# Paleogenomics/pss-bam

Measured on AMD Instinct MI355X. Metric: aligned reads/s (whole node) + HBM GB/s fraction, 200M x 150bp BAM, higher is better.
Workload: dtype u64

## Files before the change

### include/pssbam_hip.h

```cpp
#ifndef PSSBAM_HIP_H
#define PSSBAM_HIP_H

#include <stddef.h>
#include <stdint.h>

#ifdef __cplusplus
extern "C" {
#endif

#define PSSBAM_ABI_VERSION 1
#define PSSBAM_MAX_KLEN 15
#define PSSBAM_MAX_READ_GROUPS 4096
#define PSSBAM_MAX_LENGTH_BINS 64
#define PSSBAM_MAX_CONTIG_SETS 4096
#define PSSBAM_MAX_REPLICATES 64
#define PSSBAM_MAX_MISMATCHES 255
#define PSSBAM_MAX_INTERIOR_MARGIN 65535
#define PSSBAM_MAX_COMPOSITION 30
#define PSSBAM_MAX_SCORE_DIST 64
#define PSSBAM_MAX_SCORE_QUAL 64
#define PSSBAM_MAX_SCORE_WEIGHT 2047
#define PSSBAM_MAX_SCORE_HALF 128
#define PSSBAM_MAX_HIST_LENGTH 65535
#define PSSBAM_MAX_BASE_QUALITY 93
// ... 209 lines not shown
    uint32_t isize;
    uint64_t out_off;
    uint32_t crc;
    uint32_t status;
} pssbam_bgzf_block;

int64_t pssbam_bgzf_scan(const void *bytes, uint64_t nbytes, pssbam_bgzf_block *blocks, uint64_t max_blocks,
                         uint64_t *consumed, uint64_t *inflated_bytes);

int pssbam_bgzf_inflate_device(void *hip_stream, const void *d_comp, uint64_t comp_bytes, pssbam_bgzf_block *d_blocks,
                               uint32_t n_blocks, void *d_out, int check_crc);

int pssbam_engine_submit_bgzf(pssbam_engine *e, const void *comp, uint64_t comp_bytes, const pssbam_bgzf_block *blocks,
                              uint32_t n_blocks, uint32_t first_record_offset, uint64_t *ticket);
int pssbam_engine_wait_bgzf_copied(pssbam_engine *e, uint64_t ticket);
int pssbam_engine_feed_open(pssbam_engine *e, int32_t n_ref, uint64_t genome_bytes_hint);
int pssbam_engine_feed_break(pssbam_engine *e);
int pssbam_engine_feed_handoff(pssbam_engine *from, pssbam_engine *to);
#define PSSBAM_FEED_BAD_BLOCK 1u
#define PSSBAM_FEED_RAGGED 2u
#define PSSBAM_FEED_BAD_RECORD 4u
#define PSSBAM_FEED_TRUNCATED 8u
int pssbam_engine_feed_status(pssbam_engine *e, uint32_t *flags, double *inflate_ms, uint64_t *inflated_bytes);
int pssbam_engine_hint_records(pssbam_engine *e, const void *records, uint64_t nbytes);
int pssbam_feed_reserve(int device);
int pssbam_feed_release(int device);

int pssbam_bgzf_inflate_host(int device, const void *bgzf, uint64_t nbytes, void *out, uint64_t out_cap, uint64_t *out_len,
                             uint32_t *n_blocks, uint32_t *first_bad_block, uint32_t *first_bad_status, double *kernel_ms,
                             int check_crc, int repeats);

uint64_t pssbam_bgzf_deflate_work_bytes(uint64_t raw_bytes);
int pssbam_bgzf_deflate_device(void *hip_stream, const void *d_raw, uint64_t raw_bytes, void *d_bgzf, uint64_t bgzf_cap,
                               uint64_t *d_totals, void *d_work, uint64_t work_bytes);

int pssbam_bgzf_deflate_host(int device, const void *raw, uint64_t nbytes, void *out, uint64_t out_cap, uint64_t *out_len,
                             uint32_t *n_blocks, double *kernel_ms, int repeats);

int64_t pssbam_index_records(const void *bytes, uint64_t nbytes, uint32_t *offsets,
                             uint64_t max_records, uint64_t *consumed);

#ifdef __cplusplus
}
#endif
#endif
```

### pss-bam_amd/__init__.py

```python
from __future__ import annotations

import ctypes as C
import subprocess
from dataclasses import dataclass
from pathlib import Path

import numpy as np

PKG_DIR = Path(__file__).resolve().parent
ROOT = PKG_DIR.parent
LIB_HIP = PKG_DIR / "libpssbam_hip.so"
LIB_HOST = PKG_DIR / "libpssbam_host.so"
LIB_SYNTH = PKG_DIR / "libpssbam_synth.so"

TALLY_PSS, TALLY_KMER = 1, 2
KERNEL_AUTO, KERNEL_SIMPLE, KERNEL_TILED = 0, 1, 2
ST_NAMES = ["records", "rg_dropped", "parse_skip", "no_contig", "pss_ok", "pss_filtered", "kmer_ok",
            "kmer_filtered", "kmer_fail", "slow_path"]
ST_N = 16

HIP_SYMBOLS = [
    "pssbam_last_error", "pssbam_device_count", "pssbam_warmup", "pssbam_engine_create", "pssbam_engine_destroy",
    "pssbam_engine_set_stream", "pssbam_engine_set_genome", "pssbam_engine_set_genome_arrays",
    "pssbam_engine_set_references", "pssbam_engine_submit", "pssbam_engine_submit_async", "pssbam_engine_wait_copied",
    "pssbam_engine_copy_done", "pssbam_engine_phase_times", "pssbam_engine_submit_device", "pssbam_engine_sync",
    "pssbam_engine_finish", "pssbam_engine_reset", "pssbam_engine_counters_device", "pssbam_engine_bind_counters",
    "pssbam_reduce_counters", "pssbam_engine_genome_kmer_count", "pssbam_host_register", "pssbam_host_unregister", "pssbam_engine_timer_begin",
    "pssbam_engine_timer_end", "pssbam_engine_kernel_time", "pssbam_index_records", "pssbam_bgzf_scan",
    "pssbam_bgzf_inflate_device", "pssbam_bgzf_inflate_host", "pssbam_engine_submit_bgzf", "pssbam_engine_wait_bgzf_copied",
    "pssbam_engine_feed_status", "pssbam_engine_feed_break", "pssbam_engine_feed_handoff", "pssbam_feed_reserve", "pssbam_engine_hint_records",
    "pssbam_engine_set_genome_async", "pssbam_engine_genome_wait", "pssbam_engine_feed_open", "pssbam_feed_release",
    "pssbam_engine_set_read_groups", "pssbam_engine_finish_groups", "pssbam_engine_set_length_bins",
    "pssbam_engine_set_contig_sets", "pssbam_engine_finish_kmer_groups", "pssbam_engine_set_min_base_quality",
    "pssbam_engine_set_regions", "pssbam_engine_set_length_histogram", "pssbam_engine_finish_length_histogram",
    "pssbam_engine_set_site_context", "pssbam_engine_finish_site_context",
    "pssbam_engine_set_end_condition", "pssbam_engine_finish_end_condition", "pssbam_engine_set_gapped_reads",
    "pssbam_engine_set_per_contig", "pssbam_engine_finish_contigs",
    "pssbam_engine_set_mismatches", "pssbam_engine_finish_mismatches", "pssbam_engine_set_replicates",
    "pssbam_engine_set_interior", "pssbam_engine_finish_interior",
    "pssbam_engine_set_composition", "pssbam_engine_finish_composition",
    "pssbam_engine_set_read_score", "pssbam_engine_finish_read_score",
    "pssbam_engine_set_record_sink", "pssbam_engine_set_block_sink", "pssbam_engine_set_end_mask",
    "pssbam_engine_set_duplicates", "pssbam_engine_finish_duplicates",
    "pssbam_engine_set_coverage", "pssbam_engine_finish_coverage", "pssbam_engine_finish_coverage_runs",
    "pssbam_engine_set_sites", "pssbam_engine_finish_sites",
    "pssbam_bgzf_deflate_work_bytes", "pssbam_bgzf_deflate_device", "pssbam_bgzf_deflate_host",
]
MAX_READ_GROUPS = 4096
MAX_LENGTH_BINS = 64
MAX_CONTIG_SETS = 4096
MAX_REPLICATES = 64
MAX_BASE_QUALITY = 93
MAX_HIST_LENGTH = 65535
# ... 764 lines not shown
            rc = L.pssbam_engine_submit_bgzf(self._h, bgzf.ctypes.data + base_in, end_in - base_in, grp, j - i, skip, C.byref(t))
            if rc == EBUSY and on_busy is not None:
                on_busy()
                rc = L.pssbam_engine_submit_bgzf(self._h, bgzf.ctypes.data + base_in, end_in - base_in, grp, j - i, skip, C.byref(t))
            _chk(rc)
            _chk(L.pssbam_engine_wait_bgzf_copied(self._h, t.value))
            skip = 0
            i = j
        return int(n)

    def feed_break(self):
        self._L.pssbam_engine_feed_break.argtypes = [C.c_void_p]
        _chk(self._L.pssbam_engine_feed_break(self._h))

    def feed_handoff(self, to: "Engine"):
        self._L.pssbam_engine_feed_handoff.argtypes = [C.c_void_p, C.c_void_p]
        _chk(self._L.pssbam_engine_feed_handoff(self._h, to._h))

    def feed_status(self) -> dict:
        L = self._L
        L.pssbam_engine_feed_status.argtypes = [C.c_void_p, C.POINTER(C.c_uint32), C.POINTER(C.c_double), C.POINTER(C.c_uint64)]
        f, ms, nb = C.c_uint32(), C.c_double(), C.c_uint64()
        _chk(L.pssbam_engine_feed_status(self._h, C.byref(f), C.byref(ms), C.byref(nb)))
        return {"flags": int(f.value), "inflate_ms": float(ms.value), "inflated_bytes": int(nb.value)}

    def submit_device(self, d_records: int, nbytes: int, d_offsets: int, n_records: int):
        _chk(self._L.pssbam_engine_submit_device(self._h, C.c_void_p(d_records), nbytes, C.c_void_p(d_offsets),
                                                 n_records))

    def sync(self):
        _chk(self._L.pssbam_engine_sync(self._h))

    def reset(self):
        _chk(self._L.pssbam_engine_reset(self._h))

    def finish(self) -> Tables:
        fwd = rev = k5 = k3 = None
        if self.has_pss:
            fwd = np.zeros((self.region_len + 2, 16), dtype=np.uint64)
            rev = np.zeros_like(fwd)
        if self.has_kmer:
            k5 = np.zeros(4 ** self.klen, dtype=np.uint64)
            k3 = np.zeros_like(k5)
        st = np.zeros(ST_N, dtype=np.uint64)
        p = lambda a: a.ctypes.data if a is not None else None
        _chk(self._L.pssbam_engine_finish(self._h, p(fwd), p(rev), p(k5), p(k3), st.ctypes.data))
        return Tables(fwd, rev, k5, k3, {n: int(st[i]) for i, n in enumerate(ST_NAMES)})
# ... 96 lines not shown
```

### pss-bam_amd/csrc/bgzf_api.h

```cpp
#pragma once

#include "inflate_kernels.h"
#include "inflate_wave.h"

extern "C" int64_t pssbam_bgzf_scan(const void *bytes, uint64_t nbytes, pssbam_bgzf_block *blocks, uint64_t max_blocks,
                                    uint64_t *consumed, uint64_t *inflated_bytes) {
    const uint8_t *p = (const uint8_t *)bytes;
    uint64_t o = 0, n = 0, uoff = 0;
    while (o + 18 <= nbytes && (!blocks || n < max_blocks)) {
        if (p[o] != 0x1f || p[o + 1] != 0x8b || p[o + 2] != 8 || !(p[o + 3] & 4)) { fail(PSSBAM_EFORMAT, "not a BGZF block at offset %llu", (unsigned long long)o); return PSSBAM_EFORMAT; }
        const uint32_t xlen = p[o + 10] | ((uint32_t)p[o + 11] << 8);
        if (o + 12 + xlen > nbytes) break;
        uint32_t bsize = 0;
        bool found = false;
        for (uint32_t x = 0; x + 4 <= xlen;) {
            const uint8_t *sf = p + o + 12 + x;
            const uint32_t slen = sf[2] | ((uint32_t)sf[3] << 8);
            if (sf[0] == 'B' && sf[1] == 'C' && slen == 2 && x + 6 <= xlen) { bsize = (sf[4] | ((uint32_t)sf[5] << 8)) + 1u; found = true; break; }
            x += 4 + slen;
        }
        if (!found || bsize < 12u + xlen + 8u) { fail(PSSBAM_EFORMAT, "BGZF block at offset %llu has no usable BC field", (unsigned long long)o); return PSSBAM_EFORMAT; }
        if (o + bsize > nbytes) break;
        uint32_t crc, isize;
        memcpy(&crc, p + o + bsize - 8, 4);
        memcpy(&isize, p + o + bsize - 4, 4);
        if (isize > 65536u) { fail(PSSBAM_EFORMAT, "BGZF ISIZE %u exceeds 64 KiB", isize); return PSSBAM_EFORMAT; }
// ... 100 lines not shown
        if (!crc2_attr_set[dev & 63]) {
            HIP_TRY(hipFuncSetAttribute((const void *)pssbam::bgzf_crc_lines_kernel, hipFuncAttributeMaxDynamicSharedMemorySize, (int)pssbam::CRC2_LDS_BYTES));
            crc2_attr_set[dev & 63] = true;
        }
        const uint32_t cgrid = std::min<uint32_t>((n_blocks + 15) / 16, (uint32_t)n_cu);
        hipLaunchKernelGGL(pssbam::bgzf_crc_lines_kernel, dim3(cgrid), dim3(1024), pssbam::CRC2_LDS_BYTES, st, (const uint8_t *)d_out, (pssbam::BgzfBlock *)d_blocks, n_blocks,
                           (const uint32_t *)xpow16, (const uint32_t *)ztab);
        HIP_TRY(hipGetLastError());
        return PSSBAM_OK;
    }
    if (beside_inflate) {
        const uint32_t cgrid = std::min<uint32_t>((n_blocks + 3) / 4, (uint32_t)n_cu);
        hipLaunchKernelGGL(pssbam::bgzf_crc_kernel<4u>, dim3(cgrid), dim3(256), 4u * 256u * 4u * 4u, st, (const uint8_t *)d_out, (pssbam::BgzfBlock *)d_blocks, n_blocks, xpow);
    } else {
        static const uint32_t crc_waves = getenv("PSSBAM_CRC_WAVES") ? (uint32_t)std::min(16, std::max(1, atoi(getenv("PSSBAM_CRC_WAVES")))) : 16u;
        const uint32_t cgrid = std::min<uint32_t>((n_blocks + crc_waves - 1) / crc_waves, (uint32_t)n_cu);
        hipLaunchKernelGGL(pssbam::bgzf_crc_kernel<pssbam::CRC_REP>, dim3(cgrid), dim3(64 * crc_waves), pssbam::CRC_LDS_BYTES, st, (const uint8_t *)d_out, (pssbam::BgzfBlock *)d_blocks, n_blocks, xpow);
    }
    HIP_TRY(hipGetLastError());
    return PSSBAM_OK;
}

static int launch_inflate(hipStream_t st, const void *d_comp, uint64_t comp_bytes, pssbam_bgzf_block *d_blocks, uint32_t n_blocks,
                          void *d_out, int check_crc, int loop, uint64_t out_bytes, const WaveBufs *wb = nullptr) {
    if (!n_blocks) return PSSBAM_OK;
    if (!d_comp || !d_blocks || !d_out) return fail(PSSBAM_EINVAL, "null buffer");
    if ((uintptr_t)d_comp & 3u) return fail(PSSBAM_EINVAL, "d_comp must be 4-byte aligned");
    int dev = 0, n_cu = 0;
    HIP_TRY(hipGetDevice(&dev));
    HIP_TRY(hipDeviceGetAttribute(&n_cu, hipDeviceAttributeMultiprocessorCount, dev));
    static bool attr_set[64] = {false};
    if (!attr_set[dev & 63]) {
        HIP_TRY(hipFuncSetAttribute((const void *)pssbam::bgzf_inflate_kernel<false>, hipFuncAttributeMaxDynamicSharedMemorySize, (int)pssbam::INF_LDS_BYTES));
        HIP_TRY(hipFuncSetAttribute((const void *)pssbam::bgzf_inflate_kernel<true>, hipFuncAttributeMaxDynamicSharedMemorySize, (int)pssbam::INF_LDS_BYTES_DEFER));
        HIP_TRY(hipFuncSetAttribute((const void *)pssbam::bgzf_inflate_kernel<true, true>, hipFuncAttributeMaxDynamicSharedMemorySize, (int)pssbam::INF_LDS_BYTES_DEFER));
        HIP_TRY(hipFuncSetAttribute((const void *)pssbam::bgzf_inflate_kernel<true, true, true>, hipFuncAttributeMaxDynamicSharedMemorySize, (int)pssbam::INF_LDS_BYTES_DEFER));
        HIP_TRY(hipFuncSetAttribute((const void *)pssbam::bgzf_inflate_kernel<true, false, true>, hipFuncAttributeMaxDynamicSharedMemorySize, (int)pssbam::INF_LDS_BYTES_DEFER));
        attr_set[dev & 63] = true;
    }
    if (loop == -2) loop = 0;
    else if (const char *lm = getenv("PSSBAM_INFLATE_LOOP")) loop = atoi(lm) != 0;
    if (comp_bytes < 64u) loop = 0;
    const uint32_t groups = (n_blocks + pssbam::INF_WAVE - 1) / pssbam::INF_WAVE;
    const char *gm = getenv("PSSBAM_INFLATE_WAVES_PER_CU");
    const uint32_t per_cu = gm && atoi(gm) > 0 ? (uint32_t)atoi(gm) : (uint32_t)pssbam::INF_WAVES_PER_CU;
    const uint32_t grid = std::min<uint32_t>(groups, (uint32_t)n_cu * per_cu);
    uint32_t lit_run = out_bytes && out_bytes >= 8ull * comp_bytes ? 4u : 8u;
// ... 10 lines not shown
            if (!d_dbg2) HIP_TRY(hipMalloc(&d_dbg2, 20 * sizeof(unsigned long long)));
            HIP_TRY(hipMemsetAsync(d_dbg2, 0, 20 * sizeof(unsigned long long), st));
            d_wdbg = d_dbg2;
        }
        hipLaunchKernelGGL(pssbam::bgzf_tokens_kernel, dim3(tgrid), dim3(64 * pssbam::WV_WAVES), 0, st, (const uint8_t *)d_comp, comp_bytes, (pssbam::BgzfBlock *)d_blocks,
                           n_blocks, (uint8_t *)d_out, wb->seq_arena, wb->seq_off, wb->seq_count, d_wdbg);
        const char *rg = getenv("PSSBAM_RESOLVE_WGS_PER_CU");
        const uint32_t rgrid = std::min<uint32_t>((n_blocks + pssbam::RS_WAVES - 1) / pssbam::RS_WAVES, (uint32_t)n_cu * (rg && atoi(rg) > 0 ? (uint32_t)atoi(rg) : 4u));
        hipLaunchKernelGGL(pssbam::bgzf_resolve_kernel, dim3(rgrid), dim3(64 * pssbam::RS_WAVES), 0, st, (uint8_t *)d_out, (pssbam::BgzfBlock *)d_blocks, n_blocks,
                           (const uint32_t *)wb->seq_arena, wb->seq_off, (const uint32_t *)wb->seq_count, d_wdbg);
        HIP_TRY(hipGetLastError());
        if (d_wdbg) {
            unsigned long long h[20];
            HIP_TRY(hipMemcpyAsync(h, d_wdbg, sizeof h, hipMemcpyDeviceToHost, st));
            HIP_TRY(hipStreamSynchronize(st));
            const double nb = (double)std::max<unsigned long long>(h[9], 1), rb = (double)std::max<unsigned long long>(h[16], 1);
            fprintf(stderr, "[pssbam] token kernel stamps, shader cycles per BGZF block (%.0f blocks, %.2f chunks each): set-up+stored %.0f, code-length walk %.0f, table builds %.0f, "
                            "walk A1 %.0f, A2 %.0f, path %.0f, B+scans %.0f, C %.0f\n", nb, h[8] / nb, h[0] / nb, h[1] / nb, h[2] / nb, h[3] / nb, h[4] / nb, h[5] / nb, h[6] / nb, h[7] / nb);
            fprintf(stderr, "[pssbam] resolve kernel stamps, shader cycles per BGZF block (%.0f blocks, %.1f batches and %.1f rounds each): window in %.0f, scans %.0f, rounds %.0f, window out %.0f\n",
                    rb, h[14] / rb, h[15] / rb, h[10] / rb, h[11] / rb, h[12] / rb, h[13] / rb);
        }
        only_status = pssbam::INF_RETRY;
    }
    if (loop > 0 && getenv("PSSBAM_INFLATE_STAMPS")) {
        static unsigned long long *d_dbg = nullptr;
        if (!d_dbg) HIP_TRY(hipMalloc(&d_dbg, 8 * sizeof(unsigned long long)));
        HIP_TRY(hipMemsetAsync(d_dbg, 0, 8 * sizeof(unsigned long long), st));
        if (pieces)
            hipLaunchKernelGGL((pssbam::bgzf_inflate_kernel<true, true, true>), dim3(grid), dim3(pssbam::INF_WAVE), pssbam::INF_LDS_BYTES_DEFER, st, (const uint8_t *)d_comp,
                               comp_bytes, (pssbam::BgzfBlock *)d_blocks, n_blocks, (uint8_t *)d_out, lit_run, d_dbg);
        else
            hipLaunchKernelGGL((pssbam::bgzf_inflate_kernel<true, false, true>), dim3(grid), dim3(pssbam::INF_WAVE), pssbam::INF_LDS_BYTES_DEFER, st, (const uint8_t *)d_comp,
                               comp_bytes, (pssbam::BgzfBlock *)d_blocks, n_blocks, (uint8_t *)d_out, lit_run, d_dbg);
        unsigned long long h[8];
        HIP_TRY(hipMemcpyAsync(h, d_dbg, sizeof h, hipMemcpyDeviceToHost, st));
        HIP_TRY(hipStreamSynchronize(st));
        const double L = (double)std::max<unsigned long long>(h[3], 1);
        fprintf(stderr, "[pssbam] inflate stamps (pieces %d; lane sums, shader cycles): steps %llu, per step: decode %.0f wait %.0f stores+copies %.0f cycles; lanes in a step %.1f of 64; "
                        "literals per step %.2f; steps ending in an in-place copy %.3f; in-loop share of the lanes' kernel cycles %.3f\n", (int)pieces,
                h[3], h[0] / L, h[1] / L, h[2] / L, h[4] / L, h[5] / L, h[6] / L, (double)(h[0] + h[1] + h[2]) / (double)std::max<unsigned long long>(h[7], 1));
    } else if (only_status != 0xFFFFFFFFu && getenv("PSSBAM_INFLATE_WAVE") && atoi(getenv("PSSBAM_INFLATE_WAVE")) == 2) {
    } else if (loop > 0 && pieces)
        hipLaunchKernelGGL((pssbam::bgzf_inflate_kernel<true, true>), dim3(grid), dim3(pssbam::INF_WAVE), pssbam::INF_LDS_BYTES_DEFER, st, (const uint8_t *)d_comp,
                           comp_bytes, (pssbam::BgzfBlock *)d_blocks, n_blocks, (uint8_t *)d_out, lit_run, (unsigned long long *)nullptr, only_status);
    else if (loop > 0)
        hipLaunchKernelGGL(pssbam::bgzf_inflate_kernel<true>, dim3(grid), dim3(pssbam::INF_WAVE), pssbam::INF_LDS_BYTES_DEFER, st, (const uint8_t *)d_comp,
                           comp_bytes, (pssbam::BgzfBlock *)d_blocks, n_blocks, (uint8_t *)d_out, lit_run);
    else
        hipLaunchKernelGGL(pssbam::bgzf_inflate_kernel<false>, dim3(grid), dim3(pssbam::INF_WAVE), pssbam::INF_LDS_BYTES, st, (const uint8_t *)d_comp,
                           comp_bytes, (pssbam::BgzfBlock *)d_blocks, n_blocks, (uint8_t *)d_out, lit_run);
    HIP_TRY(hipGetLastError());
    if (check_crc) return launch_crc(st, d_blocks, n_blocks, d_out);
    return PSSBAM_OK;
}

extern "C" int pssbam_bgzf_inflate_device(void *hip_stream, const void *d_comp, uint64_t comp_bytes, pssbam_bgzf_block *d_blocks,
                                          uint32_t n_blocks, void *d_out, int check_crc) {
    return launch_inflate((hipStream_t)hip_stream, d_comp, comp_bytes, d_blocks, n_blocks, d_out, check_crc, -2, 0);
}


extern "C" int pssbam_bgzf_inflate_host(int device, const void *bgzf, uint64_t nbytes, void *out, uint64_t out_cap, uint64_t *out_len,
                                        uint32_t *n_blocks_out, uint32_t *first_bad_block, uint32_t *first_bad_status, double *kernel_ms,
                                        int check_crc, int repeats) {
    uint64_t consumed = 0, total = 0;
    const int64_t n = pssbam_bgzf_scan(bgzf, nbytes, nullptr, 0, &consumed, &total);
    if (n < 0) return (int)n;
    if (consumed != nbytes) return fail(PSSBAM_EFORMAT, "input ends inside a BGZF block");
    if (out_len) *out_len = total;
    if (n_blocks_out) *n_blocks_out = (uint32_t)n;
    if (first_bad_block) *first_bad_block = 0xFFFFFFFFu;
    if (first_bad_status) *first_bad_status = 0;
    if (n == 0) return PSSBAM_OK;
// ... 437 lines not shown
    HIP_TRY(hipStreamWaitEvent(is, s.copies_done, 0));
    HIP_TRY(hipStreamWaitEvent(is, s.copies_done2, 0));
    if (s.h_blocks_cap < nb) {
        if (s.h_blocks) (void)hipHostFree(s.h_blocks);
        s.h_blocks = nullptr;
        s.h_blocks_cap = 0;
        const size_t cap = std::max<size_t>(nb + nb / 4, 1u << 16);
        if (hipHostMalloc((void **)&s.h_blocks, cap * sizeof(pssbam_bgzf_block), hipHostMallocDefault) == hipSuccess) s.h_blocks_cap = cap;
        else s.h_blocks = nullptr;
    }
    const pssbam_bgzf_block *table = s.blocks.data();
    if (s.h_blocks) {
        memcpy(s.h_blocks, s.blocks.data(), nb * sizeof(pssbam_bgzf_block));
        table = s.h_blocks;
    }
    HIP_TRY(hipMemcpyAsync(s.d_blocks, table, nb * sizeof(pssbam_bgzf_block), hipMemcpyHostToDevice, is));
    hipEvent_t ev0 = take_event(e), ev1 = take_event(e);
    if (!ev0 || !ev1) return fail(PSSBAM_EHIP, "hipEventCreate failed");
    if (!e->feed_base_ev) {
        HIP_TRY(hipEventCreate(&e->feed_base_ev));
        HIP_TRY(hipEventRecord(e->feed_base_ev, is));
    }
    HIP_TRY(hipEventRecord(ev0, is));
    rc = launch_inflate(is, s.d_comp, s.comp_used, (pssbam_bgzf_block *)s.d_blocks, (uint32_t)nb, s.d_out, 0, INFLATE_LOOP_DEFAULT, data_end - FEED_GAP);
    if (rc) return rc;
    if (!s.inflate_done) HIP_TRY(hipEventCreateWithFlags(&s.inflate_done, hipEventDisableTiming));
    HIP_TRY(hipEventRecord(s.inflate_done, is));
    HIP_TRY(hipStreamWaitEvent(e->stream, s.inflate_done, 0));
    if (e->feed_fresh) {
        const uint64_t first = FEED_GAP + e->feed_skip;
        HIP_TRY(hipMemcpyAsync(s.d_chain, &first, sizeof first, hipMemcpyHostToDevice, e->stream));
        e->feed_fresh = false;
    } else {
        hipLaunchKernelGGL(pssbam::bgzf_chain_carry_in, dim3(1), dim3(256), 0, e->stream, (const uint8_t *)e->d_carry, (const uint64_t *)e->d_feed_tail,
                           s.d_out, (uint64_t)FEED_GAP, s.d_chain);
    }
    if (!getenv("PSSBAM_NO_CRC")) {
        rc = launch_crc(e->stream, (pssbam_bgzf_block *)s.d_blocks, (uint32_t)nb, s.d_out, is != e->stream && !getenv("PSSBAM_FEED_BIG_CRC"));
        if (rc) return rc;
    }
    const int32_t n_ref = e->have_refs ? e->n_ref : e->feed_n_ref;
    {
        const uint32_t n = (uint32_t)nb, grid = std::min<uint32_t>((n + 255u) / 256u, (uint32_t)e->n_cu * 8u);
        const pssbam::BgzfBlock *blk = (const pssbam::BgzfBlock *)s.d_blocks;
        hipLaunchKernelGGL(pssbam::bgzf_chain_spec, dim3(grid), dim3(256), 0, e->stream, (const uint8_t *)s.d_out, blk, n, data_end,
                           (const uint64_t *)s.d_chain, n_ref, s.d_a, s.d_n, s.d_e, s.d_last, e->d_feed_flags, s.d_chain + 2);
        hipLaunchKernelGGL(pssbam::bgzf_chain_suffix, dim3(1), dim3(1024), 0, e->stream, (const uint64_t *)s.d_a, n, s.d_nexta, (const uint64_t *)nullptr);
// ... 71 lines not shown
            s.sub_bytes = 0;
        }
        b.in_off = b.in_off - byte0 + comp_at;
        b.out_off = s.out_used;
        b.status = 0;
        s.out_used += b.isize;
        s.sub_bytes += b.isize;
        s.blocks.push_back(b);
    }
    HIP_TRY(hipMemcpyAsync(s.d_comp + comp_at, comp + byte0, byte1 - byte0, hipMemcpyHostToDevice, cs));
    s.comp_used = comp_at + (byte1 - byte0);
    e->h2d_bytes += byte1 - byte0;
    return PSSBAM_OK;
}

static int feed_state_init(pssbam_engine *e) {
    if (e->d_feed_flags) return PSSBAM_OK;
    e->feed_t0 = feed_now();
    if (getenv("PSSBAM_FEED_SUPER_BYTES")) e->feed_out_target = std::max<uint64_t>(1ull << 20, strtoull(getenv("PSSBAM_FEED_SUPER_BYTES"), nullptr, 10));
    if (getenv("PSSBAM_FEED_SUB_BYTES")) e->feed_sub_max = std::min<uint64_t>(FEED_SUB_MAX, std::max<uint64_t>(65536, strtoull(getenv("PSSBAM_FEED_SUB_BYTES"), nullptr, 10)));
    const uint64_t lanes = (uint64_t)e->n_cu * (uint64_t)pssbam::INF_WAVES_PER_CU * 64ull;
    const uint64_t rounds = std::max<uint64_t>(1, e->feed_out_target / (lanes * 65280ull));
    e->feed_block_target = getenv("PSSBAM_FEED_SUPER_BYTES") && e->feed_out_target < lanes * 65280ull ? 0xFFFFFFFFull : rounds * lanes;
    HIP_TRY(hipMalloc(&e->d_feed_flags, sizeof(uint32_t)));
    HIP_TRY(hipMemsetAsync(e->d_feed_flags, 0, sizeof(uint32_t), e->stream));
    HIP_TRY(hipMalloc(&e->d_feed_tail, sizeof(uint64_t)));
    HIP_TRY(hipMemsetAsync(e->d_feed_tail, 0, sizeof(uint64_t), e->stream));
    if (!e->d_carry) HIP_TRY(hipMalloc(&e->d_carry, FEED_GAP));
    if (const char *ib = getenv("PSSBAM_FEED_IDLE_BLOCKS")) e->feed_idle_min_blocks = atoi(ib) > 0 ? (uint64_t)atoi(ib) : ~0ull;
    return PSSBAM_OK;
}

extern "C" int pssbam_engine_feed_open(pssbam_engine *e, int32_t n_ref, uint64_t genome_bytes_hint) {
    if (!e || n_ref < 0) return fail(PSSBAM_EINVAL, "bad argument");
    if (e->cfg.kernel == PSSBAM_KERNEL_SIMPLE) return fail(PSSBAM_EINVAL, "device-indexed blocks need the tiled kernels");
    HIP_TRY(hipSetDevice(e->device));
    if (e->per_contig && !e->have_refs)
        if (const int rc = size_per_contig(e, n_ref)) return rc;
    e->feed_opened = true;
    e->feed_n_ref = n_ref;
    size_t free_b = 0, total_b = 0;
    if (hipMemGetInfo(&free_b, &total_b) == hipSuccess) {
        const uint64_t keep = genome_bytes_hint + genome_bytes_hint / 2 + (8ull << 30) + select_reserve_bytes(e) + dedup_reserve_bytes(e) + coverage_reserve_bytes(e);
        e->feed_mem_budget = e->feed.size() * feed_slot_bytes(e) + (free_b > keep ? free_b - keep : 0);
    }
    return PSSBAM_OK;
}

// ... 141 lines not shown
    to->feed_skip = 0;
    return PSSBAM_OK;
}

extern "C" int pssbam_engine_wait_bgzf_copied(pssbam_engine *e, uint64_t ticket) {
    if (!e) return fail(PSSBAM_EINVAL, "null engine");
    if (!ticket) return PSSBAM_OK;
    for (size_t i = 0; i < e->feed_copies.size(); i++)
        if (e->feed_copies[i].first == ticket) {
            HIP_TRY(hipSetDevice(e->device));
            HIP_TRY(hipEventSynchronize(e->feed_copies[i].second));
            e->feed_event_pool.push_back(e->feed_copies[i].second);
            e->feed_copies.erase(e->feed_copies.begin() + (long)i);
            return PSSBAM_OK;
        }
    return PSSBAM_OK;
}

extern "C" int pssbam_engine_feed_status(pssbam_engine *e, uint32_t *flags, double *inflate_ms, uint64_t *inflated_bytes) {
    if (!e) return fail(PSSBAM_EINVAL, "null engine");
    int rc = pssbam_engine_sync(e);
    if (rc) return rc;
    uint32_t f = 0;
    if (e->d_feed_flags) HIP_TRY(hipMemcpy(&f, e->d_feed_flags, sizeof f, hipMemcpyDeviceToHost));
    if (e->d_feed_tail) {
        uint64_t tail = 0;
        HIP_TRY(hipMemcpy(&tail, e->d_feed_tail, sizeof tail, hipMemcpyDeviceToHost));
        if (tail) f |= pssbam::FEED_TRUNCATED;
    }
    {
        std::vector<std::pair<float, float>> iv;
        for (auto &p : e->inflate_events) {
            float a = 0.f, b = 0.f;
            HIP_TRY(hipEventElapsedTime(&a, e->feed_base_ev, p.first));
            HIP_TRY(hipEventElapsedTime(&b, e->feed_base_ev, p.second));
            iv.emplace_back(a, b);
            e->event_pool.push_back(p.first);
            e->event_pool.push_back(p.second);
        }
        e->inflate_events.clear();
        std::sort(iv.begin(), iv.end());
        float hi = -1e30f;
        for (auto &x : iv) {
            if (x.second <= hi) continue;
            e->inflate_ms += x.second - std::max(x.first, hi);
            hi = x.second;
        }
        if (e->feed_base_ev) { (void)hipEventDestroy(e->feed_base_ev); e->feed_base_ev = nullptr; }
    }
    if (getenv("PSSBAM_STATS"))
        fprintf(stderr, "[pssbam] engine feed: %llu super-batches (%llu cut short because the device had run dry; their blocks filled %.0f %% of the lanes of the inflate launches) in %zu slots (%llu allocated here), %llu tally launches put off until the genome was set; "
                        "buffer allocation %.3f, waiting for a busy slot %.3f, flush (block table + launches) %.3f s; first launch %.3f s after the first block came\n",
                (unsigned long long)e->flush_seq, (unsigned long long)e->feed_early_flushes,
                e->feed_lanes_launched ? 100.0 * (double)e->feed_blocks_launched / (double)e->feed_lanes_launched : 0.0, e->feed.size(), (unsigned long long)e->feed_slots_allocated, (unsigned long long)e->feed_deferred_launches,
                e->feed_t_alloc, e->feed_t_wait_busy, e->feed_t_flush, e->feed_t_first_flush);
    if (flags) *flags = f;
    if (inflate_ms) *inflate_ms = e->inflate_ms;
    if (inflated_bytes) *inflated_bytes = e->inflated_bytes;
    return PSSBAM_OK;
}
```

### pss-bam_amd/csrc/engine.hip

```cpp
#include "../../include/pssbam_hip.h"
#include "../../include/fasta-genome-io.h"

#include <hip/hip_runtime.h>

#include <algorithm>
#include <condition_variable>
#include <cstdarg>
#include <cstdio>
#include <cstdlib>
#include <cstring>
#include <ctime>
#include <map>
#include <string>
#include <thread>
#include <tuple>
#include <type_traits>
#include <unordered_map>
#include <unordered_set>
#include <atomic>
#include <memory>
#include <mutex>
#include <vector>

#include "tally_kernels.h"
// ... 278 lines not shown
    double h2d_ms = 0.0;
    uint64_t h2d_bytes = 0;
    std::vector<FeedAcc *> feed;
    int cur_feed = -1, spare_feed = -1;
    uint64_t flush_seq = 0;
    bool feed_opened = false;
    int32_t feed_n_ref = 0;
    uint64_t feed_mem_budget = 0;
    std::vector<DeferredTally> deferred;
    uint8_t *d_carry = nullptr;
    uint8_t *h_handoff = nullptr;
    hipEvent_t handoff_ev = nullptr;
    uint64_t feed_out_target = FEED_OUT_TARGET, feed_comp_cap = FEED_COMP_CAP;
    uint64_t feed_sub_max = FEED_SUB_MAX;
    double feed_t_alloc = 0, feed_t_wait_busy = 0, feed_t_flush = 0;
    double feed_t0 = 0, feed_t_first_flush = -1;
    uint64_t feed_slots_allocated = 0, feed_deferred_launches = 0, feed_early_flushes = 0;
    uint64_t feed_blocks_launched = 0, feed_lanes_launched = 0;
    uint64_t feed_idle_min_blocks = 8192;
    uint64_t feed_block_target = 0;
    std::vector<std::pair<uint64_t, hipEvent_t>> feed_copies;
    std::vector<hipEvent_t> feed_event_pool;
    uint32_t *d_feed_flags = nullptr;
    uint64_t *d_feed_tail = nullptr;
    bool feed_fresh = true;
    uint32_t feed_skip = 0;
    double inflate_ms = 0.0;
    uint64_t inflated_bytes = 0;
    std::vector<std::pair<hipEvent_t, hipEvent_t>> inflate_events;
    hipEvent_t t_begin = nullptr, t_end = nullptr;
    std::vector<std::pair<hipEvent_t, hipEvent_t>> launch_events;
    std::vector<hipEvent_t> event_pool;
    double kernel_ms = 0.0;
    uint64_t kernel_launches = 0;
    int env_tile_reads = 0, env_grid_mult = 0, env_simple_blocks = 0, env_grid_wgs = 0, env_pieces = 0;
    int env_group_slots = 0;
    bool warned_ablate = false;
    bool compact_plan_once = false;
    std::unordered_map<const void *, KernelPrep> prep;
    bool use_compact = true;
    uint32_t *d_scratch = nullptr;
    size_t scratch_slots = 0;
    uint32_t dev_pieces = 0;
    uint64_t dev_pieces_avg = 0;
};

// ... 2152 lines not shown
        if (rev) for (size_t k = 0; k < tab; k++) rev[i * tab + k] = (unsigned long)p[tab + k];
    });
}

extern "C" int pssbam_engine_reset(pssbam_engine *e) {
    if (!e) return fail(PSSBAM_EINVAL, "null engine");
    HIP_TRY(hipSetDevice(e->device));
    if (!e->sel_queue.empty())
        if (const int rs = select_poll(e, true)) return rs;
    if (const int rs = select_report(e)) return rs;
    e->tallied = false;
    e->feed_fresh = true;
    e->feed_skip = 0;
    if (!e->deferred.empty()) {
        e->deferred.clear();
        for (FeedAcc *sp : e->feed)
            if (sp->held) {
                sp->held = false;
                if (!sp->consumed) HIP_TRY(hipEventCreateWithFlags(&sp->consumed, hipEventDisableTiming));
                HIP_TRY(hipEventRecord(sp->consumed, e->stream));
            }
    }
    if (e->d_feed_tail) HIP_TRY(hipMemsetAsync(e->d_feed_tail, 0, sizeof(uint64_t), e->stream));
    if (e->d_feed_flags) HIP_TRY(hipMemsetAsync(e->d_feed_flags, 0, sizeof(uint32_t), e->stream));
    HIP_TRY(hipMemsetAsync(e->d_counters, 0, e->n_counters * sizeof(unsigned long long), e->stream));
    if (e->d_dedup_state) {
        const int rd = dedup_poll(e, true);
        HIP_TRY(hipMemsetAsync(e->d_dedup_state, 0, sizeof(unsigned long long), e->stream));
        if (e->d_dedup) {
            hipLaunchKernelGGL(dedup_clear, dim3(dedup_grid(e, e->dedup_cap)), dim3(256), 0, e->stream, e->d_dedup, e->dedup_cap);
            HIP_TRY(hipGetLastError());
            e->dedup_launches++;
        }
        e->dedup_known = e->dedup_known_at = e->dedup_reading_at = e->dedup_submitted = 0;
        e->dedup_seq = 0;
        if (rd) return rd;
    }
    if (e->d_cov) {
        HIP_TRY(hipMemsetAsync(e->d_cov, 0, e->cov_len * sizeof(uint32_t), e->stream));
        e->cov_totals_valid = false;
    }
    if (e->d_site_counts)
        HIP_TRY(hipMemsetAsync(e->d_site_counts, 0, e->site_idx.size() * ALLELE_WORDS * sizeof(uint32_t), e->stream));
    return PSSBAM_OK;
}

extern "C" int pssbam_engine_finish_sites(pssbam_engine *e, uint64_t cap, int32_t *ref, uint32_t *pos0, uint8_t *ref_base, uint32_t *counts,
// ... 572 lines not shown
```

### pss-bam_amd/host/device_feed.c

```c
#include "device_feed.h"

#include <errno.h>
#include <fcntl.h>
#include <pthread.h>
#include <stdatomic.h>
#include <stdio.h>
#include <stdlib.h>
#include <string.h>
#include <sys/stat.h>
#include <time.h>
#include <unistd.h>

static double mono_s(void)
{
    struct timespec ts;
    clock_gettime(CLOCK_MONOTONIC, &ts);
    return ts.tv_sec + ts.tv_nsec * 1e-9;
}

#define MAX_STAGE 40
#define BLOCKS_PER_SCAN 65536u
#define OVER ((size_t)128 << 10)

typedef struct {
// ... 349 lines not shown
                submitted_from_chunk++;
                while (fifo_len > max_inflight || fifo_len >= 127) RETIRE();
                i = j;
            }
        }
        if (!submitted_from_chunk) {
            pthread_mutex_lock(&L->mu);
            s->free_for = k + L->n_st;
            s->loaded = -1;
            pthread_cond_broadcast(&L->cv);
            pthread_mutex_unlock(&L->mu);
        }
    }
    while (fifo_len > 0) RETIRE();
#undef RETIRE
    if (pos != L->file_size) { fprintf(stderr, "Error: %s: truncated BGZF block at end of file\n", path); goto done; }
    if (!gate_open) {
        const double tg = mono_s();
        if (gate->poll(gate->ctx, 1) <= 0) goto done;
        t_gate += mono_s() - tg;
        gate_open = 1;
    }
    fs->n_submits = n_submits;
    for (int g = 0; g < n_gpus; g++) {
        uint32_t f = 0;
        double ms = 0;
        uint64_t ib = 0;
        if (pssbam_engine_feed_status(eng[g], &f, &ms, &ib)) { fprintf(stderr, "Error: GPU engine %d: %s\n", g, pssbam_last_error()); goto done; }
        fs->flags |= f;
        fs->inflate_ms += ms;
        fs->inflated_bytes += ib;
    }
    if (fs->flags & (PSSBAM_FEED_RAGGED | PSSBAM_FEED_BAD_RECORD)) fs->fallback = 1;
    else if (fs->flags & PSSBAM_FEED_BAD_BLOCK) { fprintf(stderr, "Error: %s: BGZF inflate / CRC check failed\n", path); goto done; }
    else if (fs->flags & PSSBAM_FEED_TRUNCATED) { fprintf(stderr, "Error: %s: truncated alignment record at end of file\n", path); goto done; }
    if (verbose)
        fprintf(stderr, "[pssbam] device feed: %llu submits, %.2f GB compressed over PCIe, %.2f GB inflated on the device in %.3f s "
                        "of kernel time (%.1f GB/s), %d loader threads, %d staging slots of %zu MiB%s\n",
                (unsigned long long)n_submits, fs->compressed_bytes * 1e-9, fs->inflated_bytes * 1e-9, fs->inflate_ms * 1e-3,
                fs->inflate_ms > 0 ? fs->inflated_bytes * 1e-6 / fs->inflate_ms : 0.0, n_th, L->n_st, L->W >> 20,
                fs->fallback ? "; records cross BGZF blocks -> host reader" : "");
    if (verbose && n_gpus > 1) {
        fprintf(stderr, "[pssbam] device feed, submits per engine:");
        for (int g = 0; g < n_gpus; g++) fprintf(stderr, " %llu", (unsigned long long)submits_of[g & 63]);
        fputc('\n', stderr);
    }
    if (verbose)
        fprintf(stderr, "[pssbam] device feed, this thread: waiting for loaders %.3f, block-header walk %.3f (%ld of %ld windows walked by "
                        "their loader), submit (incl. waiting for a free slot) %.3f, waiting for copies %.3f, waiting for the genome %.3f s "
                        "(%llu of the submits went in ahead of it); first submit %.3f s after the feed began (the call took %.3f s)\n", t_wait_load, t_scan,
                n_prescanned, L->n_chunks, t_submit, t_wait_copy, t_gate, (unsigned long long)n_submits_ahead, t_first_submit, t_first_submit_dur);
    rc = 0;
done:
    if (rc) {
        pthread_mutex_lock(&L->mu);
        L->stop = 1;
        pthread_cond_broadcast(&L->cv);
        pthread_mutex_unlock(&L->mu);
        for (int g = 0; g < n_gpus; g++) (void)pssbam_engine_sync(eng[g]);
    }
    if (rc == 0 && !g_retired) g_retired = F;
    else loader_close(F);
    free(blocks);
// ... 4 lines not shown
```

Before: 23.73 billion.

## Copy stored BGZF blocks with whole waves before the inflate kernel

Adds a pre-pass kernel that classifies each BGZF block. Blocks holding a single final stored (uncompressed) deflate block are copied by a full 64-lane wave using aligned 16-byte vector stores, and the rest are marked for the normal inflate kernel, which now skips already-handled blocks via the only_status filter. This moves stored blocks off the per-lane decoder, which handles them slowly. The cost is an extra launch and a pass over the block descriptors even when no block is stored, which is the usual case for compressed BAMs.

```diff
diff --git a/include/pssbam_hip.h b/include/pssbam_hip.h
--- a/include/pssbam_hip.h
+++ b/include/pssbam_hip.h
@@ -255,6 +255,7 @@
 #define PSSBAM_FEED_BAD_RECORD 4u
 #define PSSBAM_FEED_TRUNCATED 8u
 int pssbam_engine_feed_status(pssbam_engine *e, uint32_t *flags, double *inflate_ms, uint64_t *inflated_bytes);
+int pssbam_engine_feed_stored_blocks(pssbam_engine *e, uint64_t *n_blocks);
 int pssbam_engine_hint_records(pssbam_engine *e, const void *records, uint64_t nbytes);
 int pssbam_feed_reserve(int device);
 int pssbam_feed_release(int device);
diff --git a/pss-bam_amd/__init__.py b/pss-bam_amd/__init__.py
--- a/pss-bam_amd/__init__.py
+++ b/pss-bam_amd/__init__.py
@@ -28,7 +28,7 @@
     "pssbam_reduce_counters", "pssbam_engine_genome_kmer_count", "pssbam_host_register", "pssbam_host_unregister", "pssbam_engine_timer_begin",
     "pssbam_engine_timer_end", "pssbam_engine_kernel_time", "pssbam_index_records", "pssbam_bgzf_scan",
     "pssbam_bgzf_inflate_device", "pssbam_bgzf_inflate_host", "pssbam_engine_submit_bgzf", "pssbam_engine_wait_bgzf_copied",
-    "pssbam_engine_feed_status", "pssbam_engine_feed_break", "pssbam_engine_feed_handoff", "pssbam_feed_reserve", "pssbam_engine_hint_records",
+    "pssbam_engine_feed_status", "pssbam_engine_feed_stored_blocks", "pssbam_engine_feed_break", "pssbam_engine_feed_handoff", "pssbam_feed_reserve", "pssbam_engine_hint_records",
     "pssbam_engine_set_genome_async", "pssbam_engine_genome_wait", "pssbam_engine_feed_open", "pssbam_feed_release",
     "pssbam_engine_set_read_groups", "pssbam_engine_finish_groups", "pssbam_engine_set_length_bins",
     "pssbam_engine_set_contig_sets", "pssbam_engine_finish_kmer_groups", "pssbam_engine_set_min_base_quality",
@@ -839,7 +839,10 @@
         L.pssbam_engine_feed_status.argtypes = [C.c_void_p, C.POINTER(C.c_uint32), C.POINTER(C.c_double), C.POINTER(C.c_uint64)]
         f, ms, nb = C.c_uint32(), C.c_double(), C.c_uint64()
         _chk(L.pssbam_engine_feed_status(self._h, C.byref(f), C.byref(ms), C.byref(nb)))
-        return {"flags": int(f.value), "inflate_ms": float(ms.value), "inflated_bytes": int(nb.value)}
+        L.pssbam_engine_feed_stored_blocks.argtypes = [C.c_void_p, C.POINTER(C.c_uint64)]
+        ns = C.c_uint64()
+        _chk(L.pssbam_engine_feed_stored_blocks(self._h, C.byref(ns)))
+        return {"flags": int(f.value), "inflate_ms": float(ms.value), "inflated_bytes": int(nb.value), "stored_blocks": int(ns.value)}
 
     def submit_device(self, d_records: int, nbytes: int, d_offsets: int, n_records: int):
         _chk(self._L.pssbam_engine_submit_device(self._h, C.c_void_p(d_records), nbytes, C.c_void_p(d_offsets),
diff --git a/pss-bam_amd/csrc/bgzf_api.h b/pss-bam_amd/csrc/bgzf_api.h
--- a/pss-bam_amd/csrc/bgzf_api.h
+++ b/pss-bam_amd/csrc/bgzf_api.h
@@ -2,6 +2,7 @@
 
 #include "inflate_kernels.h"
 #include "inflate_wave.h"
+#include "stored_kernel.h"
 
 extern "C" int64_t pssbam_bgzf_scan(const void *bytes, uint64_t nbytes, pssbam_bgzf_block *blocks, uint64_t max_blocks,
                                     uint64_t *consumed, uint64_t *inflated_bytes) {
@@ -148,7 +149,7 @@
 }
 
 static int launch_inflate(hipStream_t st, const void *d_comp, uint64_t comp_bytes, pssbam_bgzf_block *d_blocks, uint32_t n_blocks,
-                          void *d_out, int check_crc, int loop, uint64_t out_bytes, const WaveBufs *wb = nullptr) {
+                          void *d_out, int check_crc, int loop, uint64_t out_bytes, const WaveBufs *wb = nullptr, uint32_t *d_stored_taken = nullptr) {
     if (!n_blocks) return PSSBAM_OK;
     if (!d_comp || !d_blocks || !d_out) return fail(PSSBAM_EINVAL, "null buffer");
     if ((uintptr_t)d_comp & 3u) return fail(PSSBAM_EINVAL, "d_comp must be 4-byte aligned");
@@ -205,6 +206,15 @@
         }
         only_status = pssbam::INF_RETRY;
     }
+    const bool wave_path = only_status != 0xFFFFFFFFu;
+    const char *sc = getenv("PSSBAM_STORED_COPY");
+    if ((sc ? atoi(sc) != 0 : true) && !wave_path && !getenv("PSSBAM_INFLATE_STAMPS")) {
+        const uint32_t sgrid = std::min<uint32_t>((n_blocks + pssbam::STORED_WAVES - 1) / pssbam::STORED_WAVES, (uint32_t)n_cu * 8u);
+        hipLaunchKernelGGL(pssbam::bgzf_stored_kernel, dim3(sgrid), dim3(64 * pssbam::STORED_WAVES), 0, st, (const uint8_t *)d_comp, comp_bytes,
+                           (pssbam::BgzfBlock *)d_blocks, n_blocks, (uint8_t *)d_out, d_stored_taken);
+        HIP_TRY(hipGetLastError());
+        only_status = pssbam::INF_NOT_STORED;
+    }
     if (loop > 0 && getenv("PSSBAM_INFLATE_STAMPS")) {
         static unsigned long long *d_dbg = nullptr;
         if (!d_dbg) HIP_TRY(hipMalloc(&d_dbg, 8 * sizeof(unsigned long long)));
@@ -222,16 +232,16 @@
         fprintf(stderr, "[pssbam] inflate stamps (pieces %d; lane sums, shader cycles): steps %llu, per step: decode %.0f wait %.0f stores+copies %.0f cycles; lanes in a step %.1f of 64; "
                         "literals per step %.2f; steps ending in an in-place copy %.3f; in-loop share of the lanes' kernel cycles %.3f\n", (int)pieces,
                 h[3], h[0] / L, h[1] / L, h[2] / L, h[4] / L, h[5] / L, h[6] / L, (double)(h[0] + h[1] + h[2]) / (double)std::max<unsigned long long>(h[7], 1));
-    } else if (only_status != 0xFFFFFFFFu && getenv("PSSBAM_INFLATE_WAVE") && atoi(getenv("PSSBAM_INFLATE_WAVE")) == 2) {
+    } else if (wave_path && getenv("PSSBAM_INFLATE_WAVE") && atoi(getenv("PSSBAM_INFLATE_WAVE")) == 2) {
     } else if (loop > 0 && pieces)
         hipLaunchKernelGGL((pssbam::bgzf_inflate_kernel<true, true>), dim3(grid), dim3(pssbam::INF_WAVE), pssbam::INF_LDS_BYTES_DEFER, st, (const uint8_t *)d_comp,
                            comp_bytes, (pssbam::BgzfBlock *)d_blocks, n_blocks, (uint8_t *)d_out, lit_run, (unsigned long long *)nullptr, only_status);
     else if (loop > 0)
         hipLaunchKernelGGL(pssbam::bgzf_inflate_kernel<true>, dim3(grid), dim3(pssbam::INF_WAVE), pssbam::INF_LDS_BYTES_DEFER, st, (const uint8_t *)d_comp,
-                           comp_bytes, (pssbam::BgzfBlock *)d_blocks, n_blocks, (uint8_t *)d_out, lit_run);
+                           comp_bytes, (pssbam::BgzfBlock *)d_blocks, n_blocks, (uint8_t *)d_out, lit_run, (unsigned long long *)nullptr, only_status);
     else
         hipLaunchKernelGGL(pssbam::bgzf_inflate_kernel<false>, dim3(grid), dim3(pssbam::INF_WAVE), pssbam::INF_LDS_BYTES, st, (const uint8_t *)d_comp,
-                           comp_bytes, (pssbam::BgzfBlock *)d_blocks, n_blocks, (uint8_t *)d_out, lit_run);
+                           comp_bytes, (pssbam::BgzfBlock *)d_blocks, n_blocks, (uint8_t *)d_out, lit_run, (unsigned long long *)nullptr, only_status);
     HIP_TRY(hipGetLastError());
     if (check_crc) return launch_crc(st, d_blocks, n_blocks, d_out);
     return PSSBAM_OK;
@@ -715,7 +725,8 @@
         HIP_TRY(hipEventRecord(e->feed_base_ev, is));
     }
     HIP_TRY(hipEventRecord(ev0, is));
-    rc = launch_inflate(is, s.d_comp, s.comp_used, (pssbam_bgzf_block *)s.d_blocks, (uint32_t)nb, s.d_out, 0, INFLATE_LOOP_DEFAULT, data_end - FEED_GAP);
+    rc = launch_inflate(is, s.d_comp, s.comp_used, (pssbam_bgzf_block *)s.d_blocks, (uint32_t)nb, s.d_out, 0, INFLATE_LOOP_DEFAULT, data_end - FEED_GAP, nullptr,
+                        e->d_feed_flags + 1);
     if (rc) return rc;
     if (!s.inflate_done) HIP_TRY(hipEventCreateWithFlags(&s.inflate_done, hipEventDisableTiming));
     HIP_TRY(hipEventRecord(s.inflate_done, is));
@@ -833,8 +844,8 @@
     const uint64_t lanes = (uint64_t)e->n_cu * (uint64_t)pssbam::INF_WAVES_PER_CU * 64ull;
     const uint64_t rounds = std::max<uint64_t>(1, e->feed_out_target / (lanes * 65280ull));
     e->feed_block_target = getenv("PSSBAM_FEED_SUPER_BYTES") && e->feed_out_target < lanes * 65280ull ? 0xFFFFFFFFull : rounds * lanes;
-    HIP_TRY(hipMalloc(&e->d_feed_flags, sizeof(uint32_t)));
-    HIP_TRY(hipMemsetAsync(e->d_feed_flags, 0, sizeof(uint32_t), e->stream));
+    HIP_TRY(hipMalloc(&e->d_feed_flags, 2 * sizeof(uint32_t)));
+    HIP_TRY(hipMemsetAsync(e->d_feed_flags, 0, 2 * sizeof(uint32_t), e->stream));
     HIP_TRY(hipMalloc(&e->d_feed_tail, sizeof(uint64_t)));
     HIP_TRY(hipMemsetAsync(e->d_feed_tail, 0, sizeof(uint64_t), e->stream));
     if (!e->d_carry) HIP_TRY(hipMalloc(&e->d_carry, FEED_GAP));
@@ -1022,7 +1033,12 @@
     int rc = pssbam_engine_sync(e);
     if (rc) return rc;
     uint32_t f = 0;
-    if (e->d_feed_flags) HIP_TRY(hipMemcpy(&f, e->d_feed_flags, sizeof f, hipMemcpyDeviceToHost));
+    if (e->d_feed_flags) {
+        uint32_t w[2] = {0, 0};
+        HIP_TRY(hipMemcpy(w, e->d_feed_flags, sizeof w, hipMemcpyDeviceToHost));
+        f = w[0];
+        e->feed_stored_blocks = w[1];
+    }
     if (e->d_feed_tail) {
         uint64_t tail = 0;
         HIP_TRY(hipMemcpy(&tail, e->d_feed_tail, sizeof tail, hipMemcpyDeviceToHost));
@@ -1059,3 +1075,9 @@
     if (inflated_bytes) *inflated_bytes = e->inflated_bytes;
     return PSSBAM_OK;
 }
+
+extern "C" int pssbam_engine_feed_stored_blocks(pssbam_engine *e, uint64_t *n_blocks) {
+    if (!e || !n_blocks) return fail(PSSBAM_EINVAL, "null argument");
+    *n_blocks = e->feed_stored_blocks;
+    return PSSBAM_OK;
+}
diff --git a/pss-bam_amd/csrc/engine.hip b/pss-bam_amd/csrc/engine.hip
--- a/pss-bam_amd/csrc/engine.hip
+++ b/pss-bam_amd/csrc/engine.hip
@@ -324,6 +324,7 @@
     std::vector<std::pair<uint64_t, hipEvent_t>> feed_copies;
     std::vector<hipEvent_t> feed_event_pool;
     uint32_t *d_feed_flags = nullptr;
+    uint64_t feed_stored_blocks = 0;
     uint64_t *d_feed_tail = nullptr;
     bool feed_fresh = true;
     uint32_t feed_skip = 0;
@@ -2522,7 +2523,8 @@
             }
     }
     if (e->d_feed_tail) HIP_TRY(hipMemsetAsync(e->d_feed_tail, 0, sizeof(uint64_t), e->stream));
-    if (e->d_feed_flags) HIP_TRY(hipMemsetAsync(e->d_feed_flags, 0, sizeof(uint32_t), e->stream));
+    if (e->d_feed_flags) HIP_TRY(hipMemsetAsync(e->d_feed_flags, 0, 2 * sizeof(uint32_t), e->stream));
+    e->feed_stored_blocks = 0;
     HIP_TRY(hipMemsetAsync(e->d_counters, 0, e->n_counters * sizeof(unsigned long long), e->stream));
     if (e->d_dedup_state) {
         const int rd = dedup_poll(e, true);
diff --git a/pss-bam_amd/csrc/stored_kernel.h b/pss-bam_amd/csrc/stored_kernel.h
--- /dev/null
+++ b/pss-bam_amd/csrc/stored_kernel.h
@@ -0,0 +1,30 @@
+#pragma once
+
+#include "inflate_kernels.h"
+#include "stored_plan.h"
+
+namespace pssbam {
+
+enum : uint32_t { INF_NOT_STORED = 101u };
+constexpr int STORED_WAVES = 4;
+
+__global__ void __launch_bounds__(64 * STORED_WAVES) bgzf_stored_kernel(const uint8_t *comp, uint64_t comp_bytes, BgzfBlock *blocks,
+                                                                        uint32_t n_blocks, uint8_t *out, uint32_t *taken) {
+    const uint32_t lane = threadIdx.x & 63u, wave = threadIdx.x >> 6;
+    uint32_t mine = 0;
+    for (uint32_t bi = blockIdx.x * STORED_WAVES + wave; bi < n_blocks; bi += gridDim.x * STORED_WAVES) {
+        const BgzfBlock b = blocks[bi];
+        int take = 0;
+        if (lane == 0u) {
+            if (stored_desc_ok(b.in_off, b.in_len, b.isize, comp_bytes)) take = stored_header_ok(comp + b.in_off, b.isize);
+            blocks[bi].status = take ? INF_OK : INF_NOT_STORED;
+        }
+        take = __shfl(take, 0);
+        if (!take) continue;
+        stored_copy_lane(comp + b.in_off + 5u, out + b.out_off, b.isize, lane, 64u);
+        mine++;
+    }
+    if (taken && lane == 0u && mine) atomicAdd(taken, mine);
+}
+
+}
diff --git a/pss-bam_amd/csrc/stored_plan.h b/pss-bam_amd/csrc/stored_plan.h
--- /dev/null
+++ b/pss-bam_amd/csrc/stored_plan.h
@@ -0,0 +1,60 @@
+#ifndef PSSBAM_STORED_PLAN_H
+#define PSSBAM_STORED_PLAN_H
+
+#include <stdint.h>
+
+#if defined(__HIPCC__)
+#define STORED_FN __host__ __device__ static inline
+#else
+#define STORED_FN static inline
+#endif
+
+STORED_FN int stored_desc_ok(uint64_t in_off, uint32_t in_len, uint32_t isize, uint64_t comp_bytes) {
+    if (isize > 65536u || in_off > comp_bytes || in_len > comp_bytes - in_off) return 0;
+    if (in_len < 5u) return 0;
+    return in_len - 5u == isize;
+}
+
+STORED_FN int stored_header_ok(const uint8_t *h, uint32_t isize) {
+    const uint32_t len = (uint32_t)h[1] | ((uint32_t)h[2] << 8), nlen = (uint32_t)h[3] | ((uint32_t)h[4] << 8);
+    return (h[0] & 7u) == 1u && (len ^ nlen) == 0xFFFFu && len == isize;
+}
+
+STORED_FN void stored_split(uint32_t dst_low4, uint32_t len, uint32_t *head, uint32_t *body, uint32_t *tail) {
+    uint32_t h = (16u - (dst_low4 & 15u)) & 15u;
+    if (h > len) h = len;
+    *head = h;
+    *body = (len - h) >> 4;
+    *tail = (len - h) & 15u;
+}
+
+typedef struct { uint32_t w[4]; } stored_q16;
+STORED_FN stored_q16 stored_load16(const uint8_t *p) {
+    stored_q16 v;
+    __builtin_memcpy(&v, p, 16);
+    return v;
+}
+STORED_FN void stored_store16(uint8_t *p, stored_q16 v) {
+    __builtin_memcpy(__builtin_assume_aligned(p, 16), &v, 16);
+}
+
+STORED_FN void stored_copy_lane(const uint8_t *src, uint8_t *dst, uint32_t len, uint32_t lane, uint32_t lanes) {
+    uint32_t head, body, tail;
+    stored_split((uint32_t)((uintptr_t)dst & 15u), len, &head, &body, &tail);
+    for (uint32_t i = lane; i < head; i += lanes) dst[i] = src[i];
+    const uint8_t *s = src + head;
+    uint8_t *d = dst + head;
+    uint32_t k = lane;
+    for (; k + 3u * lanes < body; k += 4u * lanes) {
+        const stored_q16 a = stored_load16(s + 16u * k), b = stored_load16(s + 16u * (k + lanes));
+        const stored_q16 c = stored_load16(s + 16u * (k + 2u * lanes)), e = stored_load16(s + 16u * (k + 3u * lanes));
+        stored_store16(d + 16u * k, a);
+        stored_store16(d + 16u * (k + lanes), b);
+        stored_store16(d + 16u * (k + 2u * lanes), c);
+        stored_store16(d + 16u * (k + 3u * lanes), e);
+    }
+    for (; k < body; k += lanes) stored_store16(d + 16u * k, stored_load16(s + 16u * k));
+    for (uint32_t i = lane; i < tail; i += lanes) d[16u * body + i] = s[16u * body + i];
+}
+
+#endif
diff --git a/pss-bam_amd/host/device_feed.c b/pss-bam_amd/host/device_feed.c
--- a/pss-bam_amd/host/device_feed.c
+++ b/pss-bam_amd/host/device_feed.c
@@ -395,6 +395,7 @@
         gate_open = 1;
     }
     fs->n_submits = n_submits;
+    uint64_t n_stored = 0;
     for (int g = 0; g < n_gpus; g++) {
         uint32_t f = 0;
         double ms = 0;
@@ -403,15 +404,17 @@
         fs->flags |= f;
         fs->inflate_ms += ms;
         fs->inflated_bytes += ib;
+        uint64_t ns = 0;
+        if (pssbam_engine_feed_stored_blocks(eng[g], &ns) == 0) n_stored += ns;
     }
     if (fs->flags & (PSSBAM_FEED_RAGGED | PSSBAM_FEED_BAD_RECORD)) fs->fallback = 1;
     else if (fs->flags & PSSBAM_FEED_BAD_BLOCK) { fprintf(stderr, "Error: %s: BGZF inflate / CRC check failed\n", path); goto done; }
     else if (fs->flags & PSSBAM_FEED_TRUNCATED) { fprintf(stderr, "Error: %s: truncated alignment record at end of file\n", path); goto done; }
     if (verbose)
         fprintf(stderr, "[pssbam] device feed: %llu submits, %.2f GB compressed over PCIe, %.2f GB inflated on the device in %.3f s "
-                        "of kernel time (%.1f GB/s), %d loader threads, %d staging slots of %zu MiB%s\n",
+                        "of kernel time (%.1f GB/s), %d loader threads, %d staging slots of %zu MiB, %llu stored blocks copied by whole waves%s\n",
                 (unsigned long long)n_submits, fs->compressed_bytes * 1e-9, fs->inflated_bytes * 1e-9, fs->inflate_ms * 1e-3,
-                fs->inflate_ms > 0 ? fs->inflated_bytes * 1e-6 / fs->inflate_ms : 0.0, n_th, L->n_st, L->W >> 20,
+                fs->inflate_ms > 0 ? fs->inflated_bytes * 1e-6 / fs->inflate_ms : 0.0, n_th, L->n_st, L->W >> 20, (unsigned long long)n_stored,
                 fs->fallback ? "; records cross BGZF blocks -> host reader" : "");
     if (verbose && n_gpus > 1) {
         fprintf(stderr, "[pssbam] device feed, submits per engine:");
diff --git a/pss-bam_amd/host/storedcheck_main.c b/pss-bam_amd/host/storedcheck_main.c
--- /dev/null
+++ b/pss-bam_amd/host/storedcheck_main.c
@@ -0,0 +1,96 @@
+#include <stdint.h>
+#include <stdio.h>
+#include <stdlib.h>
+#include <string.h>
+
+#include "stored_plan.h"
+
+static int failures = 0;
+#define CHECK(cond, ...) do { if (!(cond)) { failures++; fprintf(stderr, "FAILED: " __VA_ARGS__); fputc('\n', stderr); } } while (0)
+
+static uint8_t byte_at(uint32_t i) { return (uint8_t)(i * 2654435761u >> 24); }
+
+static uint8_t *alloc16(size_t n) {
+    void *p = NULL;
+    if (posix_memalign(&p, 16, n ? n : 1)) { perror("posix_memalign"); exit(2); }
+    return (uint8_t *)p;
+}
+
+static void copy_case(uint32_t len, uint32_t sa, uint32_t da, int guard_behind) {
+    const uint32_t in_off = sa >= 5u ? sa - 5u : sa + 11u;
+    const size_t comp_bytes = (size_t)in_off + 5u + len;
+    uint8_t *comp = alloc16(comp_bytes);
+    memset(comp, 0xEE, in_off);
+    comp[in_off] = 0x01;
+    comp[in_off + 1] = (uint8_t)len; comp[in_off + 2] = (uint8_t)(len >> 8);
+    comp[in_off + 3] = (uint8_t)~len; comp[in_off + 4] = (uint8_t)(~len >> 8);
+    for (uint32_t i = 0; i < len; i++) comp[in_off + 5u + i] = byte_at(i + len);
+    const size_t out_bytes = (size_t)da + len + (guard_behind ? 16u : 0u);
+    uint8_t *out = alloc16(out_bytes);
+    memset(out, 0xA5, out_bytes);
+    CHECK(stored_desc_ok(in_off, 5u + len, len, comp_bytes), "len %u sa %u da %u: descriptor refused", len, sa, da);
+    CHECK(stored_header_ok(comp + in_off, len), "len %u sa %u da %u: header refused", len, sa, da);
+    uint32_t head, body, tail;
+    stored_split(da, len, &head, &body, &tail);
+    CHECK(head + 16u * body + tail == len && head < 16u && tail < 16u && (len == head || ((da + head) & 15u) == 0u),
+          "len %u da %u: split %u + 16 * %u + %u", len, da, head, body, tail);
+    for (uint32_t lane = 0; lane < 64u; lane++) stored_copy_lane(comp + in_off + 5u, out + da, len, lane, 64u);
+    int same = 1;
+    for (uint32_t i = 0; i < len; i++) same &= out[da + i] == byte_at(i + len);
+    CHECK(same, "len %u sa %u da %u: output differs", len, sa, da);
+    int guards = 1;
+    for (size_t i = 0; i < da; i++) guards &= out[i] == 0xA5;
+    for (size_t i = (size_t)da + len; i < out_bytes; i++) guards &= out[i] == 0xA5;
+    CHECK(guards, "len %u sa %u da %u: a guard byte changed", len, sa, da);
+    free(comp);
+    free(out);
+}
+
+typedef struct { const char *what; uint32_t in_len, isize; uint8_t h[5]; uint64_t in_off, comp_bytes; int want; } class_case;
+
+int main(void) {
+    static const uint32_t sizes[] = {0, 1, 15, 16, 17, 63, 64, 65, 1023, 1024, 1025, 1041, 4095, 4096, 4097, 65280, 65535};
+    unsigned n_copy = 0;
+    for (size_t s = 0; s < sizeof sizes / sizeof sizes[0]; s++)
+        for (uint32_t sa = 0; sa < 16u; sa++)
+            for (uint32_t da = 0; da < 16u; da++) {
+                copy_case(sizes[s], sa, da, 1);
+                copy_case(sizes[s], sa, da, 0);
+                n_copy += 2;
+            }
+
+    const class_case cases[] = {
+        {"final stored block", 5 + 7, 7, {0x01, 7, 0, 0xF8, 0xFF}, 0, 64, 1},
+        {"padding bits set (k = 1)", 5 + 7, 7, {0x01 | 1 << 3, 7, 0, 0xF8, 0xFF}, 0, 64, 1},
+        {"padding bits set (k = 7)", 5 + 7, 7, {0x01 | 7 << 3, 7, 0, 0xF8, 0xFF}, 0, 64, 1},
+        {"padding bits set (k = 31)", 5 + 7, 7, {0x01 | 31 << 3, 7, 0, 0xF8, 0xFF}, 0, 64, 1},
+        {"LEN = 0", 5, 0, {0x01, 0, 0, 0xFF, 0xFF}, 0, 64, 1},
+        {"LEN = 65535", 5 + 65535, 65535, {0x01, 0xFF, 0xFF, 0, 0}, 3, 3 + 5 + 65535, 1},
+        {"the payload ends with the buffer", 5 + 7, 7, {0x01, 7, 0, 0xF8, 0xFF}, 52, 64, 1},
+        {"BFINAL = 0", 5 + 7, 7, {0x00, 7, 0, 0xF8, 0xFF}, 0, 64, 0},
+        {"fixed Huffman", 5 + 7, 7, {0x03, 7, 0, 0xF8, 0xFF}, 0, 64, 0},
+        {"dynamic Huffman", 5 + 7, 7, {0x05, 7, 0, 0xF8, 0xFF}, 0, 64, 0},
+        {"BTYPE = 11", 5 + 7, 7, {0x07, 7, 0, 0xF8, 0xFF}, 0, 64, 0},
+        {"LEN ^ NLEN != 0xFFFF", 5 + 7, 7, {0x01, 7, 0, 0xF9, 0xFF}, 0, 64, 0},
+        {"LEN > isize", 5 + 8, 7, {0x01, 8, 0, 0xF7, 0xFF}, 0, 64, 0},
+        {"LEN < isize", 5 + 6, 7, {0x01, 6, 0, 0xF9, 0xFF}, 0, 64, 0},
+        {"in_len == 5 + LEN - 1", 5 + 7 - 1, 7, {0x01, 7, 0, 0xF8, 0xFF}, 0, 64, 0},
+        {"in_len == 5 + LEN + 3", 5 + 7 + 3, 7, {0x01, 7, 0, 0xF8, 0xFF}, 0, 64, 0},
+        {"in_len = 4", 4, 0, {0x01, 0, 0, 0xFF, 0xFF}, 0, 64, 0},
+        {"in_len = 0", 0, 0, {0x01, 0, 0, 0xFF, 0xFF}, 0, 64, 0},
+        {"isize 65536", 5 + 65536, 65536, {0x01, 0, 0, 0xFF, 0xFF}, 0, 5 + 65536, 0},
+        {"isize above 64 KiB", 5 + 65537, 65537, {0x01, 1, 0, 0xFE, 0xFF}, 0, 5 + 65537, 0},
+        {"the payload runs past the buffer by one byte", 5 + 7, 7, {0x01, 7, 0, 0xF8, 0xFF}, 53, 64, 0},
+        {"in_off behind the buffer", 5 + 7, 7, {0x01, 7, 0, 0xF8, 0xFF}, 65, 64, 0},
+        {"in_off + in_len wraps", 5 + 7, 7, {0x01, 7, 0, 0xF8, 0xFF}, ~0ull - 3, 64, 0},
+    };
+    for (size_t c = 0; c < sizeof cases / sizeof cases[0]; c++) {
+        const class_case *k = &cases[c];
+        const int got = stored_desc_ok(k->in_off, k->in_len, k->isize, k->comp_bytes) && stored_header_ok(k->h, k->isize);
+        CHECK(got == k->want, "classification of \"%s\": %d, expected %d", k->what, got, k->want);
+    }
+    if (failures) { fprintf(stderr, "%d check(s) failed\n", failures); return 1; }
+    printf("ok: %u copies (sizes x 16 source x 16 destination alignments, with and without bytes behind the output), %zu classifications\n",
+           n_copy, sizeof cases / sizeof cases[0]);
+    return 0;
+}
```

New measurement: 23.71 billion. Within noise of the previous version (-0.1%).
